# sdfgeoff/stereo_depth_estimation

Measured on AMD Instinct MI355X. Metric: stereo pairs/s training @320x240 bf16, 1/2/4/8 MI355X; EPE vs ref, higher is better.
Workload: dtype bf16

## Files before the change

stereo_depth_estimation_amd/csrc/conv_gemm.hip:

```cpp
#include "common.h"

namespace {

constexpr int BK = 32;
constexpr int KC = BK / 8;

template <typename T> struct TileLd;
template <> struct TileLd<__bf16> {
    static constexpr int LD = BK;
    __device__ __forceinline__ static int off(int row, int chunk) {
        const int u = (row >> 2) & 3;
        return row * LD + ((chunk ^ ((u >> 1) * 3)) << 3);
    }
    __device__ __forceinline__ static int frag_off(int row, int lane, int ks) {
        return off(row, lane >> 4) + 0 * ks;
    }
};
template <> struct TileLd<float> {
    static constexpr int LD = BK + 4;
    __device__ __forceinline__ static int off(int row, int chunk) { return row * LD + chunk * 8; }
    __device__ __forceinline__ static int frag_off(int row, int lane, int ks) { return row * LD + ks * 4 + (lane >> 4); }
};

template <typename T>
// ... 312 lines not shown
        return sd_convt_fwd(*a, batch, H, W, wpack, N, kpad, bias, out0, to_stream(s));
    if (dtype == SD_BF16 && sd_convt_dgrad_ok(*a, N, epi))
        return sd_convt_dgrad(*a, batch, H, W, wpack, N, kpad, out0, nullptr, nullptr, to_stream(s));
    if (dtype == SD_BF16 && !a->pool)
        return sd_fast_conv_gemm(*a, batch, H, W, wpack, N, kpad, epi, out0, out1, n_split, bias, stats, to_stream(s));
    SD_REQUIRE(!(dtype == SD_BF16 && epi == SD_EPI_STATS),
               "sd_conv_gemm: bf16 STATS needs an unpooled source (materialise the pool with sd_bnrelu_pool)");
    if (dtype == SD_BF16) {
        IgemmArgs<__bf16> p{g, H, W, (int)M, (const __bf16*)wpack, N, kpad, cdiv(g.kchunks, KC), epi,
                            (__bf16*)out0, (__bf16*)out1, n_split, bias, stats};
        return launch_igemm(p, to_stream(s));
    }
    IgemmArgs<float> p{g, H, W, (int)M, (const float*)wpack, N, kpad, cdiv(g.kchunks, KC), epi,
                       (float*)out0, (float*)out1, n_split, bias, stats};
    return launch_igemm(p, to_stream(s));
}

static bool convt_bnsum_ok(const sd_src& a, int N) { return a.taps == 4 && sd_convt_dgrad_ok(a, N, SD_EPI_STORE); }

extern "C" int sd_conv_gemm_bnsum_ok(int dtype, const sd_src* a, int N) {
    if (dtype != SD_BF16 || !a || a->xform[0] == SD_AFFINE || a->xform[1] == SD_AFFINE) return 0;
    return sd_halo_bnsum_ok(*a, N) || convt_bnsum_ok(*a, N) ? 1 : 0;
}

extern "C" int sd_conv_gemm_bnsum_rows(const sd_src* a, int batch, int H, int W, int N) {
    if (!a) return 0;
    if (convt_bnsum_ok(*a, N)) return sd_convt_dgrad_rows(*a, batch, H, W, N);
    return sd_halo_store_rows(batch, H, W, N, a->chans[0] + a->chans[1]);
}

extern "C" const char* sd_conv_gemm_bnsum_kernel_name(const sd_src* a, int H, int W, int N) {
    if (a && convt_bnsum_ok(*a, N)) return sd_convt_dgrad_name(*a, N, true);
    if (!a || !sd_halo_bnsum_ok(*a, N)) return "";
    return sd_halo_fwd_name(H, W, N, SD_EPI_STORE, a->chans[0], a->chans[1], true);
}

extern "C" int sd_conv_gemm_bnsum(int dtype, const sd_src* a, int batch, int H, int W, const void* wpack, int N,
                                  int kpad, void* out, const void* y, const float* scale, const float* shift,
                                  const float* mean, const float* invstd, float* partials, sd_stream s) {
    if (int e = validate_src(a, "sd_conv_gemm_bnsum")) return e;
    SD_REQUIRE(sd_conv_gemm_bnsum_ok(dtype, a, N), "sd_conv_gemm_bnsum: bf16 CK = 32 halo shapes only (_ok)");
    SD_REQUIRE(batch > 0 && H > 0 && W > 0 && wpack && out && y && scale && shift && mean && invstd && partials,
               "sd_conv_gemm_bnsum: bad args");
    GatherSrc g = make_gather(*a);
    const HaloBnSum bns{y, scale, shift, mean, invstd};
    if (convt_bnsum_ok(*a, N)) {
        SD_REQUIRE(kpad % 64 == 0 && kpad >= g.kchunks * 8 && g.Hl == 2 * H && g.Wl == 2 * W,
                   "sd_conv_gemm_bnsum: kpad/grid");
        return sd_convt_dgrad(*a, batch, H, W, wpack, N, kpad, out, &bns, partials, to_stream(s));
    }
    SD_REQUIRE(kpad % 64 == 0 && kpad >= g.kchunks * 8 && g.Hl == H && g.Wl == W, "sd_conv_gemm_bnsum: kpad/grid");
    return sd_halo_conv_fwd(*a, batch, H, W, wpack, N, kpad, SD_EPI_STORE, out, nullptr, 0, partials, to_stream(s),
                            &bns);
}

extern "C" int sd_conv3x3_ex_ok(const sd_src* a, int N) {
    return a && a->taps == 9 && a->xform[0] != SD_AFFINE && a->xform[1] != SD_AFFINE && sd_halo_fwd_ok(*a, N, SD_EPI_STORE)
               ? 1
               : 0;
}

extern "C" const char* sd_conv3x3_ex_kernel_name(const sd_src* a, int H, int W, int N, int epi, int flags, int oaff) {
    if (!sd_conv3x3_ex_ok(a, N)) return "";
    return sd_halo_fwd_name(H, W, N, epi, a->chans[0], a->chans[1], false, (flags & SD_CONV_WSPLIT) != 0, oaff != 0,
                            a->xform[0] != SD_BNRELU && (a->chans[1] == 0 || a->xform[1] != SD_BNRELU));
}

// ... 32 lines not shown
```

stereo_depth_estimation_amd/csrc/conv_halo.hip:

```cpp
#include "common.h"
#include "halo_util.h"

namespace {

constexpr int CK = 32;
#ifndef WG_EXP
#define WG_EXP 0
#endif
typedef float f32x16 __attribute__((ext_vector_type(16)));

struct HaloSrc {
    const __bf16* p0;
    const __bf16* p1;
    const float *sc0, *sh0, *sc1, *sh1;
    int c0, c1, x0, x1;
    int ctot;
};
static inline HaloSrc make_halo_src(const sd_src& s) {
    HaloSrc h;
    h.p0 = (const __bf16*)s.ptr[0];
    h.p1 = (const __bf16*)s.ptr[1];
    h.sc0 = s.scale[0];
    h.sh0 = s.shift[0];
    h.sc1 = s.scale[1];
// ... 118 lines not shown
    int xcd;
    int prio;
    unsigned long long* dbg;
    const __bf16* by;
    const float *bsc, *bsh, *bmu, *bis;
    int ksplit, gblk, cps;
    int npix;
    float* part;
};

#ifndef HC_ST_AUX
#define HC_ST_AUX 2
#endif
#ifndef HC_WDMA
#define HC_WDMA 1
#endif
#ifndef HC_VR
#define HC_VR 1
#endif
__device__ __forceinline__ void stats_add(float* own, const uint4 v, const bool live) {
    const unsigned wv[4] = {live ? v.x : 0u, live ? v.y : 0u, live ? v.z : 0u, live ? v.w : 0u};
#pragma unroll
    for (int q = 0; q < 4; ++q) {
        const f32x2 x = {__uint_as_float(wv[q] << 16), __uint_as_float(wv[q] & 0xffff0000u)};
        f32x2 sm = {own[4 * q], own[4 * q + 1]}, sq = {own[4 * q + 2], own[4 * q + 3]};
        sm += x;
        sq = __builtin_elementwise_fma(x, x, sq);
        own[4 * q] = sm.x;
        own[4 * q + 1] = sm.y;
        own[4 * q + 2] = sq.x;
        own[4 * q + 3] = sq.y;
    }
}
template <bool B> struct BoolC { static constexpr bool v = B; };
constexpr int PERSIST_BLOCKS = 256;
constexpr int SBN_MAX = 1024;
constexpr int HMAX = 384;
__host__ __device__ constexpr int halo_px_cap(int RT, int CK) { return RT == 4 ? 640 : (RT == 3 && CK == 16 ? 512 : 384); }
__host__ __device__ constexpr int halo_ld(int CK) { return CK == 8 ? 8 : CK + 8; }
__host__ __device__ constexpr int wrow_ld(int CK) { return CK == 8 ? 88 : 9 * CK + 8; }
__device__ __forceinline__ int wswz(int row) { return ((row >> 2) & 1) * 2; }

template <int PPX>
__device__ __forceinline__ int ld_pixel(int item) { return (item / (8 * PPX)) * 8 + (item & 7); }
template <int PPX>
__device__ __forceinline__ int ld_piece(int item) { return (item >> 3) % PPX; }

template <int NT, int RT, int CK, bool STATS, bool WCONST, int IT, bool BNS, bool OAFF, bool RAW>
__device__ __forceinline__ void halo_conv_body(const HFwdArgs& p) {
    static_assert(!(OAFF && (STATS || BNS)), "the affine epilogue stores eval-mode outputs (no statistics)");
    constexpr int BN = 32 * NT;
    constexpr int PPX = CK / 8;
    constexpr bool M16 = CK == 32 && IT == 1 && !BNS;
    constexpr int HX_LD = halo_ld(CK), W_LD = M16 ? 9 * CK : wrow_ld(CK);
    constexpr int HPX = IT == 2 ? 384 : halo_px_cap(RT, CK);
    constexpr int HP = (HPX * PPX + 255) / 256;
    constexpr int WPIECES = BN * 9 * PPX;
    constexpr int W_PER_THREAD = (WPIECES + 255) / 256;
    static_assert(!M16 || (HP * 256 == HPX * PPX && HPX % 16 == 0), "M16: the loader pieces tile the halo exactly");
    constexpr int HALO_ITEM = M16 ? HPX * CK : HP * 256 / PPX * HX_LD;
    constexpr int HALO_ELEMS = IT * HALO_ITEM, W_ELEMS = BN * W_LD, BUF = HALO_ELEMS + W_ELEMS;
    static_assert(IT == 1 || (IT == 2 && HP * IT <= 16), "item masks fit 16 bits");
    constexpr int KS = (9 * CK + 15) / 16;
    __shared__ __attribute__((aligned(16))) __bf16 smem[2 * BUF];
    constexpr int SCR_PX = M16 ? 16 : 32;
    __shared__ __attribute__((aligned(16))) __bf16 scr[4 * SCR_PX * BN];

    const int tid = threadIdx.x, lane = tid & 63;
    const bool is_loader = (tid >> 6) >= 4;
    const int wid = (tid >> 6) & 3;
    const int bid = p.xcd ? (blockIdx.x & 7) * (gridDim.x >> 3) + (blockIdx.x >> 3) : blockIdx.x;
    const int ks = bid / p.gblk, bb = bid - ks * p.gblk;
    const int nb = bb % p.nblk, slot = bb / p.nblk;
    const int n0 = nb * BN;
    const int nc0 = (p.a.c0 + CK - 1) / CK;
    const int ncp = nc0 + (p.a.c1 + CK - 1) / CK;
    const int nch_v = p.wsplit ? 2 * ncp : ncp;
    const int c_lo = ks * p.cps;
    const int nchunks = (c_lo + p.cps < nch_v ? c_lo + p.cps : nch_v) - c_lo;
    const int wct = p.wsplit ? 2 * p.a.ctot : p.a.ctot;
    const int mvalid = p.th * p.tw;
    const int my_items = slot < p.nsp ? (p.nsp - 1 - slot) / p.gper + 1 : 0;
    const int total = (my_items + IT - 1) / IT * nchunks;
#ifndef HC_LS_N32
#define HC_LS_N32 2
#endif
// ... 403 lines not shown
#pragma unroll
    for (int i = 0; i < RT; ++i) {
        const int m = tile_T(i) * 32 + (lane & 31);
        const int hm = m / p.tw, wm = m - hm * p.tw;
        abase[i] = m < mvalid ? hm * p.hw + wm : 0;
    }
    int abase16[M16 ? 2 * RT : 1];
    if constexpr (M16) {
#pragma unroll
        for (int i = 0; i < 2 * RT; ++i) {
            const int m = tile_T(i >> 1) * 32 + (i & 1) * 16 + (lane & 15);
            const int hm = m / p.tw, wm = m - hm * p.tw;
            abase16[i] = (lane >> 4) * HPX * 8 + (m < mvalid ? hm * p.hw + wm : 0) * 8;
        }
    }
    f32x16 acc[M16 ? 1 : IT][M16 ? 1 : RT][M16 ? 1 : NT];
    f32x4 acc4[M16 ? 2 * RT : 1][M16 ? 2 * NT : 1];
    constexpr int EPR = 64 / PPP;
    constexpr int ER = 32 / EPR;
    auto swz = [](int j, int px) { return NT == 2 ? j ^ (px & 7) : j ^ ((px >> 1) & 3); };
    unsigned erel[(RT * ER + 1) / 2];
#pragma unroll
    for (int k = 0; k < (RT * ER + 1) / 2; ++k) erel[k] = 0xffffffffu;
#pragma unroll
    for (int i = 0; i < RT; ++i)
#pragma unroll
        for (int r = 0; r < ER; ++r) {
            const int m = tile_T(i) * 32 + r * EPR + lane / PPP;
            const int hm = m / p.tw, wm = m - hm * p.tw;
            const unsigned v = m < mvalid ? (unsigned)((hm << 9) | wm) : 0xffffu;
            const int k = i * ER + r;
            erel[k / 2] = (erel[k / 2] & ~(0xffffu << (16 * (k & 1)))) | (v << (16 * (k & 1)));
        }
    constexpr bool EFAST = M16 && !(NT == 2 && RT == 3);
    constexpr int NEO = EFAST ? RT * ER : 1;
    int eoff[NEO];
#pragma unroll
    for (int k = 0; k < NEO; ++k) {
        const int m = tile_T(k / ER) * 32 + (k % ER) * EPR + lane / PPP;
        const int hm = m / p.tw, wm = m - hm * p.tw;
        eoff[k] = m < mvalid ? hm * p.W + wm : -1;
    }
    __bf16* const scw = scr + wid * SCR_PX * BN;
    constexpr int NBK = BNS ? 8 : 1, NYQ = BNS ? RT * ER : 1;
    BnsK bk[NBK / 2 > 0 ? NBK / 2 : 1];
    uint4 yq[NYQ];
    if constexpr (BNS) {
        const int c = n0 + (lane % PPP) * 8;
#pragma unroll
        for (int q = 0; q < 4; ++q) {
            float v[4][2];
#pragma unroll
            for (int h = 0; h < 2; ++h) {
                const int ch = c + 2 * q + h;
                const bool cin = ch < p.N;
                v[0][h] = cin ? p.bsc[ch] : 0.f;
                v[1][h] = cin ? p.bsh[ch] : 0.f;
                v[2][h] = cin ? p.bis[ch] : 0.f;
                v[3][h] = cin ? -p.bmu[ch] * p.bis[ch] : 0.f;
            }
            bk[q].sc = f32x2{v[0][0], v[0][1]};
            bk[q].sh = f32x2{v[1][0], v[1][1]};
            bk[q].is = f32x2{v[2][0], v[2][1]};
            bk[q].nmi = f32x2{v[3][0], v[3][1]};
        }
    }
    auto prefetch_y = [&](int itm) __attribute__((always_inline)) {
        const int sp = slot + itm * p.gper;
        const int b = sp / p.tiles, tl = sp - b * p.tiles;
        const int ty = tl / p.tiles_x;
        const int h0 = ty * p.th, w0 = (tl - ty * p.tiles_x) * p.tw;
        const int hw_img = p.H * p.W;
        const __amdgpu_buffer_rsrc_t ry = __builtin_amdgcn_make_buffer_rsrc(
            (void*)(p.by + (size_t)b * hw_img * p.N), (short)0, hw_img * p.N * 2, 0x00020000);
#pragma unroll
        for (int k = 0; k < RT * ER; ++k) {
            const unsigned rel = (erel[k / 2] >> (16 * (k & 1))) & 0xffffu;
            const int h = h0 + (int)(rel >> 9), w = w0 + (int)(rel & 511u);
            const int c = n0 + (lane % PPP) * 8;
            const bool in = (rel != 0xffffu) & (h < p.H) & (w < p.W) & (c < p.N);
            const unsigned off = in ? (unsigned)((h * p.W + w) * p.N + c) * 2u : 0x80000000u;
            const auto v = __builtin_amdgcn_raw_buffer_load_b128(ry, off, 0, 0);
            yq[k] = make_uint4(v[0], v[1], v[2], v[3]);
        }
    };

    constexpr bool DG = (WG_EXP & 1024) != 0;
    unsigned long long t_cp = 0, t_ep = 0, t_br = 0, t0 = 0, t_all = DG ? __builtin_amdgcn_s_memtime() : 0;
    int cc = 0, pass = 0;
    for (int gi = 0; gi < total; ++gi) {
        if (DG) t0 = __builtin_amdgcn_s_memtime();
        if (WG_EXP & 16384) {
            asm volatile("" ::: "memory");
            __builtin_amdgcn_sched_barrier(0);
        }
        __syncthreads();
        if (DG) {
            const unsigned long long t1 = __builtin_amdgcn_s_memtime();
            t_br += t1 - t0;
            t0 = t1;
        }
        if (WG_EXP & 16384) {
            asm volatile("" ::: "memory");
            __builtin_amdgcn_sched_barrier(0);
        }
        if (cc == 0) {
            if constexpr (M16) {
#pragma unroll
                for (int i = 0; i < 2 * RT; ++i)
#pragma unroll
                    for (int t = 0; t < 2 * NT; ++t) acc4[i][t] = f32x4{0.f, 0.f, 0.f, 0.f};
            } else {
#pragma unroll
            for (int u = 0; u < IT; ++u)
#pragma unroll
            for (int i = 0; i < RT; ++i)
#pragma unroll
                for (int t = 0; t < NT; ++t)
#pragma unroll
                    for (int r = 0; r < 16; ++r) acc[u][i][t][r] = 0.f;
            }
        }
        if constexpr (BNS) {
            if (cc == nchunks - 1) prefetch_y(pass);
        }
        const __bf16* hx = smem + (gi & 1) * BUF;
        const __bf16* wl = hx + HALO_ELEMS;
#ifndef HC_PF
#define HC_PF 1
#endif
        constexpr int PF = HC_PF;
        bf16x8 af[PF + 1][IT][RT], bfr[PF + 1][NT];
        auto read_frags = [&](int step) {
            const int slot_ = step % (PF + 1);
            const int tapv = CK == 8 ? 2 * step + (lane >> 5) : step / (CK >= 16 ? CK / 16 : 1);
            const int tap = tapv < 9 ? tapv : 8;
            const int c8 = CK == 8 ? 0 : (step % (CK >= 16 ? CK / 16 : 1)) * 2 + (lane >> 5);
            const int toff = (tap / 3) * p.hw + tap % 3;
#pragma unroll
            for (int t = 0; t < NT; ++t) {
                bfr[slot_][t] = *reinterpret_cast<const bf16x8*>(wl + (t * 32 + (lane & 31)) * W_LD + tap * CK + c8 * 8);
                if (CK == 8 && tapv > 8) bfr[slot_][t] = bf16x8{};
            }
#pragma unroll
            for (int u = 0; u < IT; ++u)
#pragma unroll
            for (int i = 0; i < RT; ++i)
                af[slot_][u][i] = *reinterpret_cast<const bf16x8*>(hx + u * HALO_ITEM + (abase[i] + toff) * HX_LD + c8 * 8);
        };
        if constexpr (VR) {
          if (!(WG_EXP & 8)) {
            constexpr int R = RT, NH = R + 2, NS = 3 * NH, PV = 2;
            constexpr int HWV = 34;
            bf16x8 av[3][2];
            bf16x8 xv[PV + 1][2];
            const __bf16* const xb = hx + (lane >> 4) * HPX * 8 + (wid * RT * HWV + (lane & 15)) * 8;
            auto readA = [&](int kw, int kh) __attribute__((always_inline)) {
// ... 141 lines not shown
            const int ty = tl / p.tiles_x;
            const int h0 = ty * p.th, w0 = (tl - ty * p.tiles_x) * p.tw;
            const int hw_img = p.H * p.W;
            if constexpr (!STATS && !BNS) {
                if (p.part) {
                    float* const pk = p.part + ((size_t)ks * p.npix + (size_t)b * hw_img) * p.N;
                    auto put = [&](int m, int c, float a0, float a1, float a2, float a3) __attribute__((always_inline)) {
                        const int hm = m / p.tw, wm = m - hm * p.tw;
                        if ((m < mvalid) & (h0 + hm < p.H) & (w0 + wm < p.W) & (n0 + c < p.N))
                            *reinterpret_cast<float4*>(pk + ((size_t)(h0 + hm) * p.W + w0 + wm) * p.N + n0 + c) =
                                make_float4(a0, a1, a2, a3);
                    };
                    if constexpr (M16) {
#pragma unroll
                        for (int i2 = 0; i2 < 2 * RT; ++i2)
#pragma unroll
                            for (int t = 0; t < 2 * NT; ++t)
                                put(tile_T(i2 >> 1) * 32 + (i2 & 1) * 16 + (lane & 15), t * 16 + 4 * (lane >> 4),
                                    acc4[i2][t][0], acc4[i2][t][1], acc4[i2][t][2], acc4[i2][t][3]);
                    } else {
#pragma unroll
                        for (int i = 0; i < RT; ++i)
#pragma unroll
                            for (int t = 0; t < NT; ++t)
#pragma unroll
                                for (int g4 = 0; g4 < 4; ++g4)
                                    put(tile_T(i) * 32 + (lane & 31), t * 32 + 8 * g4 + 4 * (lane >> 5),
                                        acc[u][i][t][4 * g4], acc[u][i][t][4 * g4 + 1], acc[u][i][t][4 * g4 + 2],
                                        acc[u][i][t][4 * g4 + 3]);
                    }
                    continue;
                }
            }
            const bool split = p.epi == SD_EPI_SPLIT || p.epi == SD_EPI_SPLIT_STATS;
            const int ns = split ? p.n_split : p.N;
            const __amdgpu_buffer_rsrc_t rs0 = __builtin_amdgcn_make_buffer_rsrc(
                (void*)(p.out0 + (size_t)b * hw_img * ns), (short)0, hw_img * ns * 2, 0x00020000);
            const __amdgpu_buffer_rsrc_t rs1 = __builtin_amdgcn_make_buffer_rsrc(
                (void*)(split ? p.out1 + (size_t)b * hw_img * (p.N - ns) : p.out0), (short)0,
                split ? hw_img * (p.N - ns) * 2 : 0, 0x00020000);
            constexpr int NPART = M16 ? 2 * RT : RT;
            constexpr int RPP = M16 ? ER / 2 : ER;
            const bool inside = h0 + p.th <= p.H && w0 + p.tw <= p.W;
            const int pix0 = h0 * p.W + w0;
            auto row_out = [&](const uint4 v, const int i, const int r, auto SPL, auto INS) {
                const int j = lane % PPP;
                bool live;
                int pix;
                if constexpr (decltype(INS)::v) {
                    live = eoff[i * ER + r] >= 0;
                    pix = pix0 + eoff[i * ER + r];
                } else {
                    const unsigned rel = (erel[(i * ER + r) / 2] >> (16 * ((i * ER + r) & 1))) & 0xffffu;
                    const int h = h0 + (int)(rel >> 9), w = w0 + (int)(rel & 511u);
                    live = (rel != 0xffffu) & (h < p.H) & (w < p.W);
                    pix = h * p.W + w;
                }
                const bool in = live & !(WG_EXP & 4096);
                const int c = n0 + j * 8;
                if constexpr (BNS) {
                    bns_add(own, v, yq[i * ER + r], live, bk);
                }
                if constexpr (STATS) {
                    stats_add(own, v, live);
                }
                __attribute__((ext_vector_type(4))) unsigned data = {v.x, v.y, v.z, v.w};
                if (!SPL.v) {
                    const unsigned off = (in & (c < p.N)) ? (unsigned)(pix * p.N + c) * 2u : 0x80000000u;
                    __builtin_amdgcn_raw_buffer_store_b128(data, rs0, off, 0, HC_ST_AUX);
                } else {
                    const unsigned o0 = (in & (c < ns)) ? (unsigned)(pix * ns + c) * 2u : 0x80000000u;
                    const unsigned o1 = (in & (c >= ns) & (c < p.N)) ? (unsigned)(pix * (p.N - ns) + c - ns) * 2u
                                                                   : 0x80000000u;
                    __builtin_amdgcn_raw_buffer_store_b128(data, rs0, o0, 0, HC_ST_AUX);
                    __builtin_amdgcn_raw_buffer_store_b128(data, rs1, o1, 0, HC_ST_AUX);
                }
            };
            if constexpr (M16) {
                constexpr int EG = (NT == 2 && RT >= 3) ? 2 : NPART;
                static_assert(NPART % EG == 0, "whole groups of halves");
                auto epi16 = [&](auto SPL, auto INS) {
#pragma unroll
                  for (int g0 = 0; g0 < NPART; g0 += EG) {
                    uint4 vv[EG][RPP];
#pragma unroll
                    for (int e = 0; e < EG; ++e) {
                        const int i2 = g0 + e;
#pragma unroll
                        for (int t = 0; t < 2 * NT; ++t) {
                            bf16x4 v;
                            const int px = lane & 15, c = t * 16 + 4 * (lane >> 4);
                            if constexpr (OAFF) {
                                const float4 sc = *reinterpret_cast<const float4*>(oaff + c);
                                const float4 sh = *reinterpret_cast<const float4*>(oaff + BN + c);
                                v[0] = (__bf16)fmaf(acc4[i2][t][0], sc.x, sh.x);
                                v[1] = (__bf16)fmaf(acc4[i2][t][1], sc.y, sh.y);
                                v[2] = (__bf16)fmaf(acc4[i2][t][2], sc.z, sh.z);
                                v[3] = (__bf16)fmaf(acc4[i2][t][3], sc.w, sh.w);
                            } else {
#pragma unroll
                                for (int q = 0; q < 4; ++q) v[q] = (__bf16)acc4[i2][t][q];
                            }
                            *reinterpret_cast<uint2*>(scw + px * BN + swz(c >> 3, px) * 8 + (c & 4)) = *reinterpret_cast<uint2*>(&v);
                        }
                        asm volatile("" ::: "memory");
#pragma unroll
                        for (int rr = 0; rr < RPP; ++rr) {
                            const int px = rr * EPR + lane / PPP, j = lane % PPP;
                            vv[e][rr] = *reinterpret_cast<const uint4*>(scw + px * BN + swz(j, px) * 8);
                        }
                        asm volatile("" ::: "memory");
                    }
#pragma unroll
                    for (int e = 0; e < EG; ++e)
#pragma unroll
                        for (int rr = 0; rr < RPP; ++rr)
                            row_out(vv[e][rr], (g0 + e) >> 1, ((g0 + e) & 1) * RPP + rr, SPL, INS);
                  }
                };
                if (split) {
                    epi16(BoolC<true>{}, BoolC<false>{});
                } else if constexpr (EFAST) {
                    if (inside) epi16(BoolC<false>{}, BoolC<true>{});
                    else epi16(BoolC<false>{}, BoolC<false>{});
                } else {
                    epi16(BoolC<false>{}, BoolC<false>{});
                }
            } else {
                constexpr int TG = BNS ? 1 : (NT == 2 && RT == 4) ? 2 : RT;
#pragma unroll
            for (int i0 = 0; i0 < RT; i0 += TG) {
              uint4 rows[TG][RPP];
#pragma unroll
              for (int e = 0; e < TG; ++e) {
                const int i = i0 + e;
#pragma unroll
                for (int t = 0; t < NT; ++t) {
                    uint2 pk[4];
#pragma unroll
                    for (int g4 = 0; g4 < 4; ++g4) {
                        bf16x4 v;
                        if constexpr (OAFF) {
                            const int c = t * 32 + 8 * g4 + 4 * (lane >> 5);
                            const float4 sc = *reinterpret_cast<const float4*>(oaff + c);
                            const float4 sh = *reinterpret_cast<const float4*>(oaff + BN + c);
                            v[0] = (__bf16)fmaf(acc[u][i][t][4 * g4 + 0], sc.x, sh.x);
                            v[1] = (__bf16)fmaf(acc[u][i][t][4 * g4 + 1], sc.y, sh.y);
                            v[2] = (__bf16)fmaf(acc[u][i][t][4 * g4 + 2], sc.z, sh.z);
                            v[3] = (__bf16)fmaf(acc[u][i][t][4 * g4 + 3], sc.w, sh.w);
                        } else {
// ... 957 lines not shown
    if (halo_it_env() == 2 && N % 64 == 0 && t.ck == 32 && ctot > 32 && t.rt == 2 &&
        (t.th + 2) * (t.tw + 2) <= 384) {
        t.ck = 16;
        t.it = 2;
    }
    return t;
}

int sd_halo_store_rows(int batch, int H, int W, int N, int ctot) {
    int nblk, gper, nsp;
    halo_grid(fwd_tile(ctot, H, W, N, false), batch, H, W, N, nblk, gper, nsp);
    return gper;
}
bool sd_halo_bnsum_ok(const sd_src& a, int N) {
    if (!sd_halo_fwd_ok(a, N, SD_EPI_STORE)) return false;
    const HTile t = fwd_tile(a.chans[0] + a.chans[1], a.H, a.W, N, false);
    return t.ck == 32 && t.it == 1 && !(N != 32 && t.rt == 3);
}

static bool wconst_chunks(int nchunks) {
    static const bool two = [] {
        const char* e = getenv("SD_HALO_WC2");
        return !(e && atoi(e) == 0);
    }();
    return nchunks == 1 || (two && nchunks == 2);
}

const char* sd_halo_fwd_name(int H, int W, int N, int epi, int c0, int c1, bool bns, bool wsplit, bool oaff, bool raw) {
    static thread_local char buf[96];
    const bool stats = epi == SD_EPI_STATS || epi == SD_EPI_SPLIT_STATS;
    const HTile t = fwd_tile(c0 + c1, H, W, N, stats);
    const bool wc = wconst_chunks((cdiv(c0, t.ck) + cdiv(c1, t.ck)) * (wsplit ? 2 : 1));
    const bool wconst = t.ck == 8 ? true : (t.ck != 16 && wc);
    const bool r = raw && halo_raw_enabled() && t.ck == 32 && t.it == 1 && !bns;
    snprintf(buf, sizeof(buf), "k_halo_conv<%d, %d, %d, %s, %s, %d, %s, %s, %s>", N == 32 ? 1 : 2, t.rt, t.ck,
             stats && !oaff ? "true" : "false", wconst ? "true" : "false", t.it, bns ? "true" : "false",
             oaff ? "true" : "false", r ? "true" : "false");
    return buf;
}

__global__ __launch_bounds__(256) void k_halo_split_reduce(const float* __restrict__ part, int ksplit, long long n8, int N,
                                                           const float* __restrict__ osc, const float* __restrict__ osh,
                                                           __bf16* __restrict__ out) {
    const long long i = (long long)blockIdx.x * 256 + threadIdx.x;
    if (i >= n8) return;
    const float4* src = reinterpret_cast<const float4*>(part) + 2 * i;
    float v[8];
    {
        const float4 a = src[0], b = src[1];
        v[0] = a.x, v[1] = a.y, v[2] = a.z, v[3] = a.w, v[4] = b.x, v[5] = b.y, v[6] = b.z, v[7] = b.w;
    }
    for (int k = 1; k < ksplit; ++k) {
        const float4 a = src[(size_t)k * 2 * n8], b = src[(size_t)k * 2 * n8 + 1];
        v[0] += a.x, v[1] += a.y, v[2] += a.z, v[3] += a.w, v[4] += b.x, v[5] += b.y, v[6] += b.z, v[7] += b.w;
    }
    if (osc) {
        const int c = (int)((8 * i) % N);
#pragma unroll
        for (int j = 0; j < 8; ++j) v[j] = fmaf(v[j], osc[c + j], osh[c + j]);
    }
    bf16x8 o;
#pragma unroll
    for (int j = 0; j < 8; ++j) o[j] = (__bf16)v[j];
    reinterpret_cast<bf16x8*>(out)[i] = o;
}

struct HSplit {
// ... 6 lines not shown
        return !(e && atoi(e) == 0);
    }();
    HSplit q{1, nch_v, nblk, gper, false};
    if (!on || epi != SD_EPI_STORE || bns || t.it != 1 || t.ck == 16) return q;
    auto grid_of = [&](int nb) {
        q.nblk = nb;
        q.gper = PERSIST_BLOCKS / nb;
        if (q.gper < 1) q.gper = 1;
        if (q.gper > nsp) q.gper = nsp;
        q.ksplit = 1;
        q.cps = nch_v;
        const int gblk = q.gper * nb;
        if (gblk < 128 && nch_v >= 2) {
            int ks = PERSIST_BLOCKS / gblk;
            if (ks > nch_v) ks = nch_v;
            if (ks > 1) {
                q.cps = cdiv(nch_v, ks);
                q.ksplit = cdiv(nch_v, q.cps);
            }
        }
    };
    grid_of(nblk);
    if (N % 64 == 0 && t.ck == 32 && t.rt <= 3 && q.gper * q.nblk * q.ksplit < 128) {
        q.nt1 = true;
        grid_of(N / 32);
    }
    return q;
}

template <int NT, int RT, int CK, int IT = 1>
static void launch_halo(bool stats, bool wconst, dim3 grid, hipStream_t st, const HFwdArgs& p, bool bns = false,
                        bool raw = false) {
    constexpr bool W0 = CK == 8, W1 = CK != 16;
    if constexpr (IT == 1 && CK == 32) {
        if (raw && !bns) {
            auto go = [&](auto ST, auto WC, auto OA) {
                hipLaunchKernelGGL((k_halo_conv<NT, RT, CK, decltype(ST)::v, decltype(WC)::v, 1, false, decltype(OA)::v,
                                                true>),
                                   grid, dim3(512), 0, st, p);
            };
            auto by_wc = [&](auto ST, auto OA) {
                if (wconst) go(ST, BoolC<true>{}, OA);
                else go(ST, BoolC<false>{}, OA);
            };
            if (p.osc) by_wc(BoolC<false>{}, BoolC<true>{});
            else if (stats) by_wc(BoolC<true>{}, BoolC<false>{});
            else by_wc(BoolC<false>{}, BoolC<false>{});
            return;
        }
    }
    if constexpr (IT == 1 && CK != 16) {
        if (p.osc) {
            if (wconst ? W1 : W0)
                hipLaunchKernelGGL((k_halo_conv<NT, RT, CK, false, W1, IT, false, true>), grid, dim3(512), 0, st, p);
            else
                hipLaunchKernelGGL((k_halo_conv<NT, RT, CK, false, W0, IT, false, true>), grid, dim3(512), 0, st, p);
            return;
        }
    }
    if constexpr (CK == 32 && IT == 1 && !(NT == 2 && RT == 3)) {
        if (bns) {
            if (wconst ? W1 : W0)
                hipLaunchKernelGGL((k_halo_conv<NT, RT, CK, false, W1, IT, true>), grid, dim3(512), 0, st, p);
            else
                hipLaunchKernelGGL((k_halo_conv<NT, RT, CK, false, W0, IT, true>), grid, dim3(512), 0, st, p);
            return;
// ... 57 lines not shown
        p.by = (const __bf16*)bns->y;
        p.bsc = bns->scale;
        p.bsh = bns->shift;
        p.bmu = bns->mean;
        p.bis = bns->invstd;
    }
    const int nch = cdiv(p.a.c0, t.ck) + cdiv(p.a.c1, t.ck);
    HSplit q = halo_split_plan(t, p.nblk, p.gper, p.nsp, N, nch * (wsplit ? 2 : 1), epi, bns != nullptr);
    const long long need = q.ksplit > 1 ? (long long)q.ksplit * batch * H * W * N * 4 : 0;
    if (q.ksplit > 1 && (!ws || ws_bytes < need || ((uintptr_t)ws & 15) != 0)) {
        q.ksplit = 1;
        q.cps = nch * (wsplit ? 2 : 1);
    }
    p.nblk = q.nblk;
    p.gper = q.gper;
    p.gblk = q.gper * q.nblk;
    p.ksplit = q.ksplit;
    p.cps = q.cps;
    p.npix = batch * H * W;
    p.part = q.ksplit > 1 ? (float*)ws : nullptr;
    p.xcd = halo_xcd_enabled() && (p.gblk * q.ksplit) % 8 == 0;
    p.prio = halo_prio(a);
    p.dbg = g_wg_dbg;
    const int cap = t.it == 2 ? 384 : halo_px_cap(t.rt, t.ck);
    SD_REQUIRE(t.rt >= 2 && t.rt <= 4 && p.nhalo <= cap && t.th * t.tw <= 128 * t.rt &&
                   t.th < 64 && t.tw < 512,
               "sd_conv_gemm(halo): tile %dx%d (RT %d, CK %d)", t.th, t.tw, t.rt, t.ck);
    SD_REQUIRE((long long)batch * p.tiles < (1LL << 30), "sd_conv_gemm(halo): too many tiles");
    SD_REQUIRE((long long)H * W < (1LL << 24) && (long long)H * W * (a.chans[0] > a.chans[1] ? a.chans[0] : a.chans[1]) * 2 <
                   (1LL << 31) && (long long)N * kpad * 2 < (1LL << 31) && (long long)H * W * N * 2 < (1LL << 31),
               "sd_conv_gemm(halo): image %dx%d or weights %dx%d too large for 32-bit offsets", H, W, N, kpad);
    const dim3 grid(p.gblk * q.ksplit);
    const bool wc = wconst_chunks(q.cps);
    const bool raw = halo_raw_enabled() && t.ck == 32 && t.it == 1 && !bns && a.xform[0] != SD_BNRELU &&
                     (a.chans[1] == 0 || a.xform[1] != SD_BNRELU);
    SD_REQUIRE(!(N == 32 && t.ck == 32 && t.rt == 4) || (t.th == 16 && t.tw == 32),
               "sd_conv_gemm(halo): the N = 32 RT 4 instances (vertical reuse) need 16x32 tiles, got %dx%d", t.th, t.tw);
    SD_REQUIRE(t.ck != 8 || nch == 1, "sd_conv_gemm(halo): CK = 8 needs <= 8 input channels");
    if (q.nt1) {
        if (t.rt == 3) launch_halo<1, 3, 32>(st_, wc, grid, st, p, false, raw);
        else launch_halo<1, 2, 32>(st_, wc, grid, st, p, false, raw);
    } else if (t.ck == 8) {
        if (t.rt == 4) launch_halo<1, 4, 8>(st_, wc, grid, st, p);
        else if (t.rt == 3) launch_halo<1, 3, 8>(st_, wc, grid, st, p);
        else launch_halo<1, 2, 8>(st_, wc, grid, st, p);
    } else if (N == 32) {
        if (t.rt == 4) launch_halo<1, 4, 32>(st_, wc, grid, st, p, bns, raw);
        else if (t.rt == 3) launch_halo<1, 3, 32>(st_, wc, grid, st, p, bns, raw);
        else launch_halo<1, 2, 32>(st_, wc, grid, st, p, bns, raw);
    } else if (t.ck == 32) {
        if (t.rt == 3) launch_halo<2, 3, 32>(st_, wc, grid, st, p, bns, raw);
        else launch_halo<2, 2, 32>(st_, wc, grid, st, p, bns, raw);
    } else if (t.it == 2) {
        launch_halo<2, 2, 16, 2>(st_, wc, grid, st, p);
    } else if (t.rt == 4) {
        launch_halo<2, 4, 16>(st_, wc, grid, st, p);
    } else if (t.rt == 3) {
        launch_halo<2, 3, 16>(st_, wc, grid, st, p);
    } else {
        launch_halo<2, 2, 16>(st_, wc, grid, st, p);
    }
    if (q.ksplit > 1) {
        const long long n8 = (long long)batch * H * W * N / 8;
        hipLaunchKernelGGL(k_halo_split_reduce, dim3((unsigned)((n8 + 255) / 256)), dim3(256), 0, st, p.part, q.ksplit,
                           n8, N, osc, osh, (__bf16*)out0);
    }
    return sd_check_launch("sd_conv_gemm(halo)");
// ... 213 lines not shown
```

stereo_depth_estimation_amd/engine.py:

```python

from __future__ import annotations

import os
from dataclasses import dataclass, field

import torch

from . import _lib as L

BN_EPS = 1e-5
BN_MOMENTUM = 0.1
BLOCKS_FWD = ("enc1", "enc2", "enc3", "enc4", "bottleneck", "dec4", "dec3", "dec2", "dec1")
LEVEL = {"enc1": 0, "enc2": 1, "enc3": 2, "enc4": 3, "bottleneck": 4, "dec4": 3, "dec3": 2, "dec2": 1, "dec1": 0}
UP_OF_DEC = {"dec4": "up4", "dec3": "up3", "dec2": "up2", "dec1": "up1"}
DEC_OF_UP = {u: d for d, u in UP_OF_DEC.items()}
SKIP_OF_DEC = {"dec4": "enc4", "dec3": "enc3", "dec2": "enc2", "dec1": "enc1"}
UP_SRC = {"up4": "bottleneck", "up3": "dec4", "up2": "dec3", "up1": "dec2"}
PREV_ENC = {"enc2": "enc1", "enc3": "enc2", "enc4": "enc3", "bottleneck": "enc4"}


def _r64(x: int) -> int:
    return (x + 63) // 64 * 64


def _r16(x: int) -> int:
    return (x + 15) // 16 * 16


@dataclass
class ConvL:
    name: str
    blk: str
    idx: int
    cin: int
    cin_pad: int
    cout: int
    level: int
    w_key: str
    bn_key: str
    kpad_f: int = 0
    kpad_d: int = 0
    off_f: int = 0
    off_d: int = -1
    kpad8: int = 0
    off8: int = 0
    soff8: int = 0
    kpad_s: int = 0
    off_s: int = -1


@dataclass
# ... 105 lines not shown
            for cl in self.convs.values():
                if (cl.level == 0 or mode != "fullres") and (cl.cout == 32 or cl.cout % 64 == 0):
                    cl.kpad_s, cl.off_s = _r64(18 * cl.cin_pad), offs
                    offs += cl.cout * cl.kpad_s
            for u in self.ups.values():
                if u.name == "up1" or mode != "fullres":
                    u.kpad_s, u.off_s = _r64(2 * u.cin), offs
                    offs += 4 * u.cout * u.kpad_s
        self.wsplit_pack = torch.zeros(max(offs, 1), dtype=torch.bfloat16, device=self.device)
        if self.fp8:
            off8 = soff = 0
            for cl in self.convs.values():
                cl.kpad8 = _r64(9 * _r16(cl.cin_pad))
                cl.off8, cl.soff8 = off8, soff
                off8 += cl.cout * cl.kpad8
                soff += cl.cout
            self.wq8 = torch.zeros(off8, dtype=torch.uint8, device=self.device)
            self.wscale8 = torch.zeros(soff, dtype=torch.float32, device=self.device)
        self.c1 = c[0]
        self._q8_shapes = all((cl.cout == 32 or cl.cout % 64 == 0) and cl.cin_pad <= 512 for cl in self.convs.values()) \
            and all(u.cout % 16 == 0 for u in self.ups.values())
        dev = self.device
        self._counts = torch.zeros(2, 2, dtype=torch.int32, device=dev)
        self._cslot = 0
        self.count_local = self._counts[0, 0:1]
        self.count = self._counts[0, 1:2]
        self.metrics = torch.zeros(5, dtype=torch.float64, device=dev)
        self.adam_step = torch.zeros(1, dtype=torch.int32, device=dev)
        self.adam_scratch = torch.zeros(4, dtype=torch.float32, device=dev)
        self.ws: Workspace | None = None
        self.bn_fuse = os.environ.get("SD_BN_FUSE", "1") != "0"
        self.bias_fuse = os.environ.get("SD_BIAS_FUSE", "1") != "0"
        self.bnsum_fuse = os.environ.get("SD_BNSUM_FUSE", "1") != "0"
        self.bwd_fuse = {"0": 0, "1": 1}.get(os.environ.get("SD_BWD_FUSE", "2"), 2)
        self.prologue = os.environ.get("SD_PROLOGUE", "1") != "0"
        self._bnsum_rows: dict[str, int] = {}
        self.side_mode = int(os.environ.get("SD_SIDE_REDUCE", "0"))
        self.defer_reduce = os.environ.get("SD_DEFER_REDUCE", "1") != "0" and not self.side_mode
        self._red_jobs: list = []
        self._side: torch.cuda.Stream | None = None
        self._slab_free: list = [None, None]
        self._slab_i = 0
        self.bn_sync = None
        self._bn64: torch.Tensor | None = None
        self.params: dict[str, torch.Tensor] = {}
        self.grads: dict[str, torch.Tensor] = {}
        self.bufs: dict[str, torch.Tensor] = {}

    def bind(self, params: dict, bufs: dict, grads: dict | None = None, watch: list | None = None):
        self.params, self.bufs = params, bufs
        self.grads = grads or {}
        self._watch = watch if watch is not None else list(params.values()) + list(bufs.values())
        self._watch_inference = any(t.is_inference() for t in self._watch)
        self._bind_id = getattr(self, "_bind_id", 0) + 1
        self._buf_list = list(bufs.values())

    def _s(self):
        return L.stream_handle(self.device)

    def touch_state(self):
        self.state_epoch += 1

    def _state_key(self):
        if self._watch_inference:
            return None
        return (self.state_epoch, self._bind_id, tuple([t._version for t in self._watch]),
# ... 129 lines not shown
                ch = self._fp8_src_chans(cl) + (0,)
                dummy = L.make_src(None, ch[0], H >> cl.level, W >> cl.level, taps=9, c1=ch[1])
                for flags in (0, L.SD_CONV_WSPLIT) if cl.off_s >= 0 else (0,):
                    hws = max(hws, L.call("sd_conv3x3_ex_ws_bytes", dummy, B, H >> cl.level, W >> cl.level, cl.cout,
                                          L.SD_EPI_STORE, flags))
            t["hws"] = torch.empty(max(hws // 4, 4), dtype=f32, device=dev)
        if self.fp8:
            if train:
                raise RuntimeError("precision='fp8' is the inference-only forward (BASELINE config 5): no training")
            for cl in self.convs.values():
                rows = L.call("sd_conv3x3_fp8_rows", B, H >> cl.level, W >> cl.level, cl.cout)
                t["mm:" + cl.name] = torch.empty(rows, cl.cout, 2, dtype=f32, device=dev)
                t["as:" + cl.name] = torch.empty(1, dtype=f32, device=dev)
                for k, ch in enumerate(self._fp8_src_chans(cl)):
                    t[f"qs{k}:{cl.name}"] = torch.empty(ch, dtype=f32, device=dev)
                    t[f"qh{k}:{cl.name}"] = torch.empty(ch, dtype=f32, device=dev)
            t["mm:xin"] = torch.empty(L.call("sd_chan_minmax_rows", B * H * W, self.cin_pad0), self.cin_pad0, 2,
                                      dtype=f32, device=dev)
            for u in self.ups.values():
                P = B * (H >> (u.level - 1)) * (W >> (u.level - 1))
                t["mm:" + u.name] = torch.empty(L.call("sd_chan_minmax_rows", P, u.cout), u.cout, 2, dtype=f32,
                                                device=dev)
        if train:
            max_chan = max_slab = 0
            for cl in self.convs.values():
                lv = cl.level
                P = B * (H >> lv) * (W >> lv)
                t["da:" + cl.name] = act(lv, cl.cout)
                t["dy:" + cl.name] = act(lv, cl.cout)
                t["coef:" + cl.name] = torch.empty(cl.cout, 3, dtype=f32, device=dev)
                max_chan = max(max_chan, L.call("sd_chan_reduce_rows", P, cl.cout) * cl.cout * 2)
                if self._bwd_fused(cl, H, W) == 1:
                    max_chan = max(max_chan, L.call("sd_conv3x3_bwd_fused_splits", B, H >> lv, W >> lv) * 32 * 2)
                sp = self._conv_splits(cl, B, H, W)
                max_slab = max(max_slab, sp * cl.cout * 9 * cl.cin_pad)
            for u in self.ups.values():
                lv = u.level
                t["du:" + u.name] = act(lv - 1, u.cout)
                t["dskip:" + u.name] = act(lv - 1, u.cout)
                P = B * (H >> (lv - 1)) * (W >> (lv - 1))
                max_chan = max(max_chan, L.call("sd_chan_reduce_rows", P, u.cout) * u.cout * 2)
                sp = L.call("sd_wgrad_splits", dt, B, H >> lv, W >> lv, u.cin, 4 * u.cout)
                max_slab = max(max_slab, sp * u.cin * 4 * u.cout)
                dsrc = L.make_src(t["du:" + u.name], u.cout, H >> (lv - 1), W >> (lv - 1), taps=4)
                if L.call("sd_conv_gemm_bnsum_ok", dt, dsrc, u.cin) == 1:
                    rows = L.call("sd_conv_gemm_bnsum_rows", dsrc, B, H >> lv, W >> lv, u.cin)
                    max_chan = max(max_chan, rows * u.cin * 2)
            for blk in ("enc2", "enc3", "enc4", "bottleneck"):
                prev = self.convs[PREV_ENC[blk] + ".1"]
                t["dpool:" + blk] = act(prev.level + 1, prev.cout)
                if self._pool_bn_fused(prev):
                    rows = L.call("sd_pool_bwd_rows", B, H >> prev.level, W >> prev.level, prev.cout)
                    max_chan = max(max_chan, rows * prev.cout * 2)
            max_chan = max(max_chan, L.call("sd_heads_rows", B * H * W) * self.convs["dec1.1"].cout * 2)
            t["chan"] = torch.empty(max_chan, dtype=f32, device=dev)
            if self.defer_reduce:
                ws.slab_off = {}
                tot = 0
                for cl in self.convs.values():
                    sp = self._conv_splits(cl, B, H, W)
                    ws.slab_off[cl.name] = tot
                    tot += _r16(sp * cl.cout * 9 * cl.cin_pad)
                for u in self.ups.values():
                    lv = u.level
                    sp = L.call("sd_wgrad_splits", dt, B, H >> lv, W >> lv, u.cin, 4 * u.cout)
                    ws.slab_off[u.name] = tot
                    tot += _r16(sp * u.cin * 4 * u.cout)
                    dec0 = self.convs[DEC_OF_UP[u.name] + ".0"]
                    Hd, Wd = H >> dec0.level, W >> dec0.level
                    rows = L.call("sd_conv_gemm_stat_rows", dt, B, Hd, Wd, dec0.cin) * dec0.cin * 2
                    rows = max(rows, L.call("sd_conv3x3_bwd_fused_splits", B, Hd, Wd) * 32 * 2)
                    ws.slab_off["brows:" + u.name] = tot
                    tot += _r16(rows)
                max_slab = tot
            t["slab"] = torch.empty(max_slab, dtype=f32, device=dev)
            if self.side_mode:
                t["slab1"] = torch.empty(max_slab, dtype=f32, device=dev)
                self._slab_free = [None, None]
            P0 = B * H * W
            t["heads_part"] = torch.empty(L.call("sd_heads_rows", P0) * (2 * self.c1 + 7), dtype=f32, device=dev)
        self.ws = ws
        return ws

    def _bwd_fused(self, cl: ConvL, H: int, W: int) -> int:
        if not self.bwd_fuse or self.sd_dtype != L.SD_BF16:
            return 0
        Hl, Wl = H >> cl.level, W >> cl.level
        if cl.idx == 1 and cl.cout == 32 and cl.cin == 32 and self.bnsum_fuse:
            return 1 if L.call("sd_conv3x3_bwd_fused_ok", cl.cout, cl.cin, Hl, Wl) == 1 else 0
        if cl.idx == 0 and cl.blk in UP_OF_DEC and self.bwd_fuse >= 2:
            up, sk = self.ups[UP_OF_DEC[cl.blk]], self.convs[SKIP_OF_DEC[cl.blk] + ".1"]
            if cl.cin == up.cout + sk.cout and L.call("sd_conv3x3_bwd_fused_dec_ok", cl.cout, up.cout, sk.cout, Hl,
                                                      Wl) == 1:
                return 2
        return 0

    def _conv_splits(self, cl: ConvL, B: int, H: int, W: int) -> int:
        lv = cl.level
        sp = L.call("sd_wgrad_splits", self.sd_dtype, B, H >> lv, W >> lv, cl.cout, 9 * cl.cin_pad)
        if self._bwd_fused(cl, H, W):
            sp = max(sp, L.call("sd_conv3x3_bwd_fused_splits", B, H >> lv, W >> lv))
        return sp

    def _bn(self, cl: ConvL):
        t = self.ws.t
        if cl.name in self._zs:
            return (self._one[:cl.cout], self._zero[:cl.cout])
        return (t["scale:" + cl.name], t["shift:" + cl.name])

    def _src_fwd(self, cl: ConvL) -> L.SdSrc:
        ws, t = self.ws, self.ws.t
        Hl, Wl = ws.H >> cl.level, ws.W >> cl.level
        if cl.name == "enc1.0":
            return L.make_src(t["xin"], self.cin_pad0, Hl, Wl, taps=9)
        if cl.idx == 1:
            prev = self.convs[cl.blk + ".0"]
            return L.make_src(t["y:" + prev.name], prev.cout, Hl, Wl, taps=9, bn0=self._bn(prev))
        if cl.blk in PREV_ENC:
            prev = self.convs[PREV_ENC[cl.blk] + ".1"]
            if self.sd_dtype == L.SD_BF16:
                return L.make_src(t["pool:" + prev.name], prev.cout, Hl, Wl, taps=9)
            return L.make_src(t["y:" + prev.name], prev.cout, 2 * Hl, 2 * Wl, taps=9, pool=True, bn0=self._bn(prev))
        up = self.ups[UP_OF_DEC[cl.blk]]
        sk = self.convs[SKIP_OF_DEC[cl.blk] + ".1"]
        return L.make_src(
            t["u:" + up.name], up.cout, Hl, Wl, taps=9, src1=t["y:" + sk.name], c1=sk.cout, bn1=self._bn(sk)
        )

# ... 534 lines not shown
                    t["invstd:" + cl.name].data_ptr(), t["coef:" + cl.name].data_ptr(), t["y:" + c0.name].data_ptr(),
                    t["scale:" + c0.name].data_ptr(), t["shift:" + c0.name].data_ptr(),
                    t["mean:" + c0.name].data_ptr(), t["invstd:" + c0.name].data_ptr(), self._wp(cl.off_d),
                    cl.kpad_d, ws.B, Hl, Wl, t["da:" + c0.name].data_ptr())
            self._wgrad_slabs(lambda slab, st: L.call("sd_conv3x3_bwd_fused", *args, slab, t["chan"].data_ptr(), st),
                              sp, cl.cout, 9 * cl.cin_pad, L.SD_W_CONV3, cl.cin, self.grads[cl.w_key],
                              gemm_may_side=False, key=cl.name)
            self._bnsum_rows[c0.name] = sp
            return
        dy = t["dy:" + cl.name]
        a = L.make_src(dy, cl.cout, Hl, Wl, taps=1)
        b = self._src_fwd(cl)
        M, N = cl.cout, 9 * cl.cin_pad
        if not need_dgrad and dt == L.SD_BF16:
            a_nody = L.make_src(None, cl.cout, Hl, Wl, taps=1)
            if self.bn_fuse and L.call("sd_wgrad_bnbwd_ok", dt, a_nody, b, M, N) == 1:
                a = a_nody
        nblk = L.call("sd_wgrad_bnbwd_ok", dt, a, b, M, N) if self.bn_fuse and dt == L.SD_BF16 else 0
        fuse = nblk == 1 or (nblk == 2 and cl.level == 0)
        self._bn_bwd(cl, fused_rows, apply=not fuse)
        if fuse:
            sp = L.call("sd_wgrad_splits", dt, ws.B, Hl, Wl, M, N)
            args = (t["da:" + cl.name].data_ptr(), t["y:" + cl.name].data_ptr(), t["scale:" + cl.name].data_ptr(),
                    t["shift:" + cl.name].data_ptr(), t["mean:" + cl.name].data_ptr(),
                    t["invstd:" + cl.name].data_ptr(), t["coef:" + cl.name].data_ptr())
            self._wgrad_slabs(lambda slab, st: L.call("sd_wgrad_gemm_bnbwd", dt, a, b, ws.B, Hl, Wl, M, N, *args,
                                                      slab, sp, st),
                              sp, M, N, L.SD_W_CONV3, cl.cin, self.grads[cl.w_key], gemm_may_side=False, key=cl.name)
        if need_dgrad:
            dsrc = L.make_src(dy, cl.cout, Hl, Wl, taps=9)
            if cl.idx == 1:
                out = t["da:" + cl.blk + ".0"]
                c0 = self.convs[cl.blk + ".0"]
                if (self.bnsum_fuse and dt == L.SD_BF16 and cl.cin <= 64
                        and L.call("sd_conv_gemm_bnsum_ok", dt, dsrc, cl.cin) == 1):
                    L.call("sd_conv_gemm_bnsum", dt, dsrc, ws.B, Hl, Wl, self._wp(cl.off_d), cl.cin, cl.kpad_d,
                           out.data_ptr(), t["y:" + c0.name].data_ptr(), t["scale:" + c0.name].data_ptr(),
                           t["shift:" + c0.name].data_ptr(), t["mean:" + c0.name].data_ptr(),
                           t["invstd:" + c0.name].data_ptr(), t["chan"].data_ptr(), s)
                    self._bnsum_rows[c0.name] = L.call("sd_conv_gemm_bnsum_rows", dsrc, ws.B, Hl, Wl, cl.cin)
                else:
                    L.call("sd_conv_gemm", dt, dsrc, ws.B, Hl, Wl, self._wp(cl.off_d), cl.cin, cl.kpad_d,
                           L.SD_EPI_STORE, out.data_ptr(), None, 0, None, None, s)
            elif cl.blk in PREV_ENC:
                out = t["dpool:" + cl.blk]
                L.call("sd_conv_gemm", dt, dsrc, ws.B, Hl, Wl, self._wp(cl.off_d), cl.cin, cl.kpad_d, L.SD_EPI_STORE,
                       out.data_ptr(), None, 0, None, None, s)
            else:
                up = self.ups[UP_OF_DEC[cl.blk]]
                sums = self.bias_fuse and dt == L.SD_BF16 and (cl.cin == 32 or cl.cin % 64 == 0)
                brows = self._bias_rows_ptr(up.name) if sums else None
                L.call("sd_conv_gemm", dt, dsrc, ws.B, Hl, Wl, self._wp(cl.off_d), cl.cin, cl.kpad_d,
                       L.SD_EPI_SPLIT_STATS if sums else L.SD_EPI_SPLIT, t["du:" + up.name].data_ptr(),
                       t["dskip:" + up.name].data_ptr(), up.cout, None, brows, s)
                self._up_bias_rows = ((L.call("sd_conv_gemm_stat_rows", dt, ws.B, Hl, Wl, cl.cin), cl.cin, brows)
                                      if sums else None)
        if not fuse:
            self._wgrad(a, b, cl.level, M, N, L.SD_W_CONV3, cl.cin, self.grads[cl.w_key], cl.name)

    def _up_bwd(self, u: UpL):
        ws, t, s, dt = self.ws, self.ws.t, self._s(), self.sd_dtype
        du = t["du:" + u.name]
        Hh, Wh = ws.H >> (u.level - 1), ws.W >> (u.level - 1)
        Hl, Wl = ws.H >> u.level, ws.W >> u.level
        P = ws.B * Hh * Wh
        rows_ld = getattr(self, "_up_bias_rows", None)
        if rows_ld is not None:
# ... 76 lines not shown
```

Baseline: 7720.

## Extend fused BN-sum dgrad to deep blocks via M16 raw halo path

Lets the BN-statistics-fused dgrad halo kernel use the M16 raw MFMA path when NT=2 and RT=2, with the y prefetch moved earlier, split epilogue disabled, and scheduling barriers added to limit register pressure. The engine now also applies the fused dgrad+BN-sum to wider-channel layers in enc3/enc4/dec4/dec3, and sizes the channel-partials buffer to match. The goal is to remove separate BN-backward reduction passes and use faster MFMA tiles, at the cost of more register pressure and more partial rows for wide layers.

```diff
diff --git a/stereo_depth_estimation_amd/csrc/conv_gemm.hip b/stereo_depth_estimation_amd/csrc/conv_gemm.hip
--- a/stereo_depth_estimation_amd/csrc/conv_gemm.hip
+++ b/stereo_depth_estimation_amd/csrc/conv_gemm.hip
@@ -368,7 +368,8 @@
 extern "C" const char* sd_conv_gemm_bnsum_kernel_name(const sd_src* a, int H, int W, int N) {
     if (a && convt_bnsum_ok(*a, N)) return sd_convt_dgrad_name(*a, N, true);
     if (!a || !sd_halo_bnsum_ok(*a, N)) return "";
-    return sd_halo_fwd_name(H, W, N, SD_EPI_STORE, a->chans[0], a->chans[1], true);
+    return sd_halo_fwd_name(H, W, N, SD_EPI_STORE, a->chans[0], a->chans[1], true, false, false,
+                            a->xform[0] != SD_BNRELU && (a->chans[1] == 0 || a->xform[1] != SD_BNRELU));
 }
 
 extern "C" int sd_conv_gemm_bnsum(int dtype, const sd_src* a, int batch, int H, int W, const void* wpack, int N,
diff --git a/stereo_depth_estimation_amd/csrc/conv_halo.hip b/stereo_depth_estimation_amd/csrc/conv_halo.hip
--- a/stereo_depth_estimation_amd/csrc/conv_halo.hip
+++ b/stereo_depth_estimation_amd/csrc/conv_halo.hip
@@ -174,6 +174,7 @@
         own[4 * q + 3] = sq.y;
     }
 }
+__host__ __device__ constexpr bool bns_m16(int NT, int RT) { return NT == 2 && RT == 2; }
 template <bool B> struct BoolC { static constexpr bool v = B; };
 constexpr int PERSIST_BLOCKS = 256;
 constexpr int SBN_MAX = 1024;
@@ -193,7 +194,8 @@
     static_assert(!(OAFF && (STATS || BNS)), "the affine epilogue stores eval-mode outputs (no statistics)");
     constexpr int BN = 32 * NT;
     constexpr int PPX = CK / 8;
-    constexpr bool M16 = CK == 32 && IT == 1 && !BNS;
+    constexpr bool M16 = CK == 32 && IT == 1 && (!BNS || bns_m16(NT, RT));
+    constexpr bool BM16 = BNS && M16;
     constexpr int HX_LD = halo_ld(CK), W_LD = M16 ? 9 * CK : wrow_ld(CK);
     constexpr int HPX = IT == 2 ? 384 : halo_px_cap(RT, CK);
     constexpr int HP = (HPX * PPX + 255) / 256;
@@ -663,7 +665,7 @@
             const int k = i * ER + r;
             erel[k / 2] = (erel[k / 2] & ~(0xffffu << (16 * (k & 1)))) | (v << (16 * (k & 1)));
         }
-    constexpr bool EFAST = M16 && !(NT == 2 && RT == 3);
+    constexpr bool EFAST = M16 && !(NT == 2 && RT == 3) && !BNS;
     constexpr int NEO = EFAST ? RT * ER : 1;
     int eoff[NEO];
 #pragma unroll
@@ -696,6 +698,11 @@
             bk[q].nmi = f32x2{v[3][0], v[3][1]};
         }
     }
+    auto rel_of = [&](int k) __attribute__((always_inline)) {
+        unsigned e = erel[k / 2];
+        if constexpr (BM16) asm volatile("" : "+v"(e));
+        return (e >> (16 * (k & 1))) & 0xffffu;
+    };
     auto prefetch_y = [&](int itm) __attribute__((always_inline)) {
         const int sp = slot + itm * p.gper;
         const int b = sp / p.tiles, tl = sp - b * p.tiles;
@@ -706,7 +713,7 @@
             (void*)(p.by + (size_t)b * hw_img * p.N), (short)0, hw_img * p.N * 2, 0x00020000);
 #pragma unroll
         for (int k = 0; k < RT * ER; ++k) {
-            const unsigned rel = (erel[k / 2] >> (16 * (k & 1))) & 0xffffu;
+            const unsigned rel = rel_of(k);
             const int h = h0 + (int)(rel >> 9), w = w0 + (int)(rel & 511u);
             const int c = n0 + (lane % PPP) * 8;
             const bool in = (rel != 0xffffu) & (h < p.H) & (w < p.W) & (c < p.N);
@@ -753,7 +760,7 @@
             }
         }
         if constexpr (BNS) {
-            if (cc == nchunks - 1) prefetch_y(pass);
+            if (cc == (BM16 ? 0 : nchunks - 1)) prefetch_y(pass);
         }
         const __bf16* hx = smem + (gi & 1) * BUF;
         const __bf16* wl = hx + HALO_ELEMS;
@@ -961,7 +968,7 @@
                     continue;
                 }
             }
-            const bool split = p.epi == SD_EPI_SPLIT || p.epi == SD_EPI_SPLIT_STATS;
+            const bool split = !BM16 && (p.epi == SD_EPI_SPLIT || p.epi == SD_EPI_SPLIT_STATS);
             const int ns = split ? p.n_split : p.N;
             const __amdgpu_buffer_rsrc_t rs0 = __builtin_amdgcn_make_buffer_rsrc(
                 (void*)(p.out0 + (size_t)b * hw_img * ns), (short)0, hw_img * ns * 2, 0x00020000);
@@ -980,7 +987,7 @@
                     live = eoff[i * ER + r] >= 0;
                     pix = pix0 + eoff[i * ER + r];
                 } else {
-                    const unsigned rel = (erel[(i * ER + r) / 2] >> (16 * ((i * ER + r) & 1))) & 0xffffu;
+                    const unsigned rel = rel_of(i * ER + r);
                     const int h = h0 + (int)(rel >> 9), w = w0 + (int)(rel & 511u);
                     live = (rel != 0xffffu) & (h < p.H) & (w < p.W);
                     pix = h * p.W + w;
@@ -989,6 +996,10 @@
                 const int c = n0 + j * 8;
                 if constexpr (BNS) {
                     bns_add(own, v, yq[i * ER + r], live, bk);
+                    if constexpr (BM16) {
+#pragma unroll
+                        for (int q = 0; q < NOWN; ++q) asm volatile("" : "+v"(own[q]));
+                    }
                 }
                 if constexpr (STATS) {
                     stats_add(own, v, live);
@@ -1043,8 +1054,10 @@
 #pragma unroll
                     for (int e = 0; e < EG; ++e)
 #pragma unroll
-                        for (int rr = 0; rr < RPP; ++rr)
+                        for (int rr = 0; rr < RPP; ++rr) {
                             row_out(vv[e][rr], (g0 + e) >> 1, ((g0 + e) & 1) * RPP + rr, SPL, INS);
+                            if constexpr (BM16) __builtin_amdgcn_sched_barrier(0);
+                        }
                   }
                 };
                 if (split) {
@@ -2068,7 +2081,7 @@
     const HTile t = fwd_tile(c0 + c1, H, W, N, stats);
     const bool wc = wconst_chunks((cdiv(c0, t.ck) + cdiv(c1, t.ck)) * (wsplit ? 2 : 1));
     const bool wconst = t.ck == 8 ? true : (t.ck != 16 && wc);
-    const bool r = raw && halo_raw_enabled() && t.ck == 32 && t.it == 1 && !bns;
+    const bool r = raw && halo_raw_enabled() && t.ck == 32 && t.it == 1 && (!bns || bns_m16(N == 32 ? 1 : 2, t.rt));
     snprintf(buf, sizeof(buf), "k_halo_conv<%d, %d, %d, %s, %s, %d, %s, %s, %s>", N == 32 ? 1 : 2, t.rt, t.ck,
              stats && !oaff ? "true" : "false", wconst ? "true" : "false", t.it, bns ? "true" : "false",
              oaff ? "true" : "false", r ? "true" : "false");
@@ -2141,6 +2154,15 @@
 static void launch_halo(bool stats, bool wconst, dim3 grid, hipStream_t st, const HFwdArgs& p, bool bns = false,
                         bool raw = false) {
     constexpr bool W0 = CK == 8, W1 = CK != 16;
+    if constexpr (IT == 1 && CK == 32 && bns_m16(NT, RT)) {
+        if (raw && bns) {
+            if (wconst)
+                hipLaunchKernelGGL((k_halo_conv<NT, RT, CK, false, true, 1, true, false, true>), grid, dim3(512), 0, st, p);
+            else
+                hipLaunchKernelGGL((k_halo_conv<NT, RT, CK, false, false, 1, true, false, true>), grid, dim3(512), 0, st, p);
+            return;
+        }
+    }
     if constexpr (IT == 1 && CK == 32) {
         if (raw && !bns) {
             auto go = [&](auto ST, auto WC, auto OA) {
@@ -2264,7 +2286,8 @@
                "sd_conv_gemm(halo): image %dx%d or weights %dx%d too large for 32-bit offsets", H, W, N, kpad);
     const dim3 grid(p.gblk * q.ksplit);
     const bool wc = wconst_chunks(q.cps);
-    const bool raw = halo_raw_enabled() && t.ck == 32 && t.it == 1 && !bns && a.xform[0] != SD_BNRELU &&
+    const bool raw = halo_raw_enabled() && t.ck == 32 && t.it == 1 && (!bns || bns_m16(N == 32 ? 1 : 2, t.rt)) &&
+                     a.xform[0] != SD_BNRELU &&
                      (a.chans[1] == 0 || a.xform[1] != SD_BNRELU);
     SD_REQUIRE(!(N == 32 && t.ck == 32 && t.rt == 4) || (t.th == 16 && t.tw == 32),
                "sd_conv_gemm(halo): the N = 32 RT 4 instances (vertical reuse) need 16x32 tiles, got %dx%d", t.th, t.tw);
diff --git a/stereo_depth_estimation_amd/engine.py b/stereo_depth_estimation_amd/engine.py
--- a/stereo_depth_estimation_amd/engine.py
+++ b/stereo_depth_estimation_amd/engine.py
@@ -17,6 +17,7 @@
 SKIP_OF_DEC = {"dec4": "enc4", "dec3": "enc3", "dec2": "enc2", "dec1": "enc1"}
 UP_SRC = {"up4": "bottleneck", "up3": "dec4", "up2": "dec3", "up1": "dec2"}
 PREV_ENC = {"enc2": "enc1", "enc3": "enc2", "enc4": "enc3", "bottleneck": "enc4"}
+BNSUM_DEEP_BLOCKS = frozenset({"enc3", "enc4", "dec4", "dec3"})
 
 
 def _r64(x: int) -> int:
@@ -188,6 +189,7 @@
         self.bn_fuse = os.environ.get("SD_BN_FUSE", "1") != "0"
         self.bias_fuse = os.environ.get("SD_BIAS_FUSE", "1") != "0"
         self.bnsum_fuse = os.environ.get("SD_BNSUM_FUSE", "1") != "0"
+        self.bnsum_deep = {"0": False, "1": True}.get(os.environ.get("SD_BNSUM_DEEP", ""))
         self.bwd_fuse = {"0": 0, "1": 1}.get(os.environ.get("SD_BWD_FUSE", "2"), 2)
         self.prologue = os.environ.get("SD_PROLOGUE", "1") != "0"
         self._bnsum_rows: dict[str, int] = {}
@@ -383,6 +385,11 @@
                 max_chan = max(max_chan, L.call("sd_chan_reduce_rows", P, cl.cout) * cl.cout * 2)
                 if self._bwd_fused(cl, H, W) == 1:
                     max_chan = max(max_chan, L.call("sd_conv3x3_bwd_fused_splits", B, H >> lv, W >> lv) * 32 * 2)
+                elif cl.idx == 1 and dt == L.SD_BF16:
+                    dsrc = L.make_src(t["dy:" + cl.name], cl.cout, H >> lv, W >> lv, taps=9)
+                    if L.call("sd_conv_gemm_bnsum_ok", dt, dsrc, cl.cin) == 1:
+                        rows = L.call("sd_conv_gemm_bnsum_rows", dsrc, B, H >> lv, W >> lv, cl.cin)
+                        max_chan = max(max_chan, rows * cl.cin * 2)
                 sp = self._conv_splits(cl, B, H, W)
                 max_slab = max(max_slab, sp * cl.cout * 9 * cl.cin_pad)
             for u in self.ups.values():
@@ -445,6 +452,11 @@
                                                       Wl) == 1:
                 return 2
         return 0
+
+    def _bnsum_dgrad(self, cl: ConvL) -> bool:
+        if cl.cin <= 64:
+            return True
+        return cl.blk in BNSUM_DEEP_BLOCKS if self.bnsum_deep is None else self.bnsum_deep
 
     def _conv_splits(self, cl: ConvL, B: int, H: int, W: int) -> int:
         lv = cl.level
@@ -1045,7 +1057,7 @@
             if cl.idx == 1:
                 out = t["da:" + cl.blk + ".0"]
                 c0 = self.convs[cl.blk + ".0"]
-                if (self.bnsum_fuse and dt == L.SD_BF16 and cl.cin <= 64
+                if (self.bnsum_fuse and dt == L.SD_BF16 and self._bnsum_dgrad(cl)
                         and L.call("sd_conv_gemm_bnsum_ok", dt, dsrc, cl.cin) == 1):
                     L.call("sd_conv_gemm_bnsum", dt, dsrc, ws.B, Hl, Wl, self._wp(cl.off_d), cl.cin, cl.kpad_d,
                            out.data_ptr(), t["y:" + c0.name].data_ptr(), t["scale:" + c0.name].data_ptr(),
```

Measured after the change: 7726, median of 2. About the same (+0.1%).
